# hanruihua/NeuPAN

Measured on AMD Instinct MI355X. Metric: MPC plans/sec (node), diff robot, 1k pts, T=10, K=10; ctrl L2 vs ref, higher is better.
Workload: dtype f32; 1 GPU; BASELINE.json configs[1]: batch=256 synthetic scenes/GPU, diff robot, 1000 pts, T=10, K=10 (iter_threshold=0), M=10, fp32 DUNE (MFMA) + fp64 QP; scenes_per_gpu=256, points=1000, T=10, K=10, M=10, batches_in_flight=40, chains=8, issue_threads=8

## Files before the change

### neupan_amd/csrc/create.hip

```cpp
#include "handle.h"
#include "launch.h"

#include <algorithm>
#include <cmath>
#include <cstdio>
#include <cstdlib>
#include <cstring>
#include <map>

static std::mutex g_pack_mu;
static std::map<std::string, std::weak_ptr<SharedPack>> g_packs;
static long long g_pack_calibrations = 0, g_pack_hits = 0;

struct CalibKnobDef { const char* name; void (*parse)(const char* v, CalibKnobs& k); };
static Precision parse_precision(const char* v) {
  return !strcmp(v, "bf16") ? Precision::bf16 : (!strcmp(v, "fp32") ? Precision::fp32 : Precision::invalid);
}
static const CalibKnobDef kCalibKnobs[] = {
    {"NPA_DUNE_FP32KEYS", [](const char*, CalibKnobs& k) { k.forced_mode = 0; }},
    {"NPA_KEY_TERMS", [](const char* v, CalibKnobs& k) { const int t = atoi(v); if (k.forced_mode != 0 && (t == 1 || t == 3 || t == 4)) k.forced_mode = t; }},
    {"NPA_KEY_SAFETY", [](const char* v, CalibKnobs& k) { const double s = atof(v); if (s >= 1.0 && s <= 1e3) k.key_safety = s; }},
    {"NPA_GEO_GRID", [](const char* v, CalibKnobs& k) { const int n = atoi(v); if (n >= 64 && n <= 8192) k.geo_grid = n / 8 * 8; }},
    {"NPA_GEO_NOCHECK", [](const char*, CalibKnobs& k) { k.geo_nocheck = true; }},
    {"NPA_GEO_TABLE", [](const char* v, CalibKnobs& k) { k.geo_table = atoi(v) != 0; }},
    {"NPA_KTAB_SAFETY", [](const char* v, CalibKnobs& k) { const double s = atof(v); if (s >= 1.0 && s <= 100.0) k.ktab_safety = s; }},
    {"NPA_KEYS_PRECISION", [](const char* v, CalibKnobs& k) { k.keys_precision = parse_precision(v); }},
    {"NPA_K16_SAFETY", [](const char* v, CalibKnobs& k) { const double s = atof(v); if (s >= 1.0 && s <= 100.0) k.k16_safety = s; }},
    {"NPA_ROWS_PRECISION", [](const char* v, CalibKnobs& k) { k.rows_precision = parse_precision(v); }},
};

struct Knobs {
  CalibKnobs calib;
  std::string calib_key;
  bool sel_debug = false, qp_cold = false, qp_generic = false, skip_selftest = false, pack_cache = true;
  bool qp_order = true;
  double audit_rate = 1.0 / 64.0;
  float margin_scale = 1.f;
};

static Knobs read_knobs() {
  Knobs k;
  for (const CalibKnobDef& d : kCalibKnobs) {
    const char* v = getenv(d.name);
    k.calib_key.push_back('|');
    if (v) { k.calib_key.append(v); d.parse(v, k.calib); } else k.calib_key.push_back('\x01');
  }
  k.sel_debug = getenv("NPA_SEL_DEBUG") != nullptr;
  k.qp_cold = getenv("NPA_QP_COLD") != nullptr;
  k.qp_generic = getenv("NPA_QP_GENERIC") != nullptr;
  if (const char* env = getenv("NPA_QP_ORDER")) k.qp_order = atoi(env) != 0;
  k.skip_selftest = getenv("NPA_SKIP_SELFTEST") != nullptr;
  if (const char* env = getenv("NPA_PACK_CACHE")) k.pack_cache = atoi(env) != 0;
  if (const char* env = getenv("NPA_AUDIT_RATE")) { double v = atof(env); if (v >= 0.0 && v <= 1.0) k.audit_rate = v; }
  if (const char* env = getenv("NPA_GEO_MARGIN_SCALE")) { double v = atof(env); if (v > 0.0 && v <= 100.0) k.margin_scale = (float)v; }
  return k;
}

#ifdef NPA_EXPERIMENTS
static void read_experiment_knobs(npa_handle* h) { h->select_v1 = getenv("NPA_SELECT_V1") != nullptr; }
#endif


template <class T>
struct DevScratch {
  T* p = nullptr;
  hipError_t alloc_zeroed(size_t n) {
    hipError_t e = hipMalloc(&p, n * sizeof(T));
    return e == hipSuccess ? hipMemset(p, 0, n * sizeof(T)) : e;
  }
  ~DevScratch() { if (p) (void)hipFree(p); }
};

static void set_calibrated(DevParams& P, const Calibration& c) { P.geo_rcal = c.geo_rcal; P.geo_far = c.geo_far; P.geo_tab = c.geo_tab; }

static void use_key_mode(npa_handle* h) { h->key_terms = h->cal.key_terms; h->key_err = h->cal.key_err; h->key_e0 = h->cal.key_e0; }
static void apply_calibration(npa_handle* h, const Calibration& c) {
  h->cal = c;
  set_calibrated(h->P, c);
  use_key_mode(h);
}

static constexpr int kBandsPadded = (NPA_GEO_BANDS + 3) & ~3;
static const float kCalibHalves[3] = {8.f, 32.f, 128.f};

static void band_margins(const float* raw, const bool* seen, double safety, float floor, float* margin, float* near) {
  for (int bnd = 0; bnd < NPA_GEO_BANDS; ++bnd) {
    float m = -1.f;
    for (int q = std::max(bnd - 1, 0); q <= std::min(bnd + 1, NPA_GEO_BANDS - 1); ++q)
      if (seen[q]) m = std::max(m, raw[q]);
    near[bnd] = m;
    margin[bnd] = (m < 0.f || !(m < 1e30f)) ? INFINITY : std::max((float)(safety * m), floor);
  }
}

static void residual_margins(const unsigned* bits, double safety, float floor, float (&margin)[kBandsPadded], float& worst_err,
                             float& worst_margin) {
  float raw[NPA_GEO_BANDS], near[NPA_GEO_BANDS];
  bool seen[NPA_GEO_BANDS];
  for (int bnd = 0; bnd < NPA_GEO_BANDS; ++bnd) { memcpy(&raw[bnd], &bits[bnd], 4); seen[bnd] = bits[bnd] != 0u; }
  for (int bnd = 0; bnd < kBandsPadded; ++bnd) margin[bnd] = INFINITY;
  band_margins(raw, seen, safety, floor, margin, near);
  worst_err = 0.f; worst_margin = 0.f;
  for (int bnd = 0; bnd <= npa_geo_band(8.0f) && bnd < NPA_GEO_BANDS; ++bnd)
    if (near[bnd] >= 0.f) { worst_err = std::max(worst_err, near[bnd]); worst_margin = std::max(worst_margin, margin[bnd]); }
}

static hipError_t calibrate_network_keys(const DevParams& P, const float* wpack, const CalibKnobs& k, int forced, Calibration& c) {
  const int modes[2] = {1, 3};
  const float floor_e0[2] = {1e-4f, 2e-5f}, cap_e0[2] = {5e-2f, 1e-3f};
  bool ok[2] = {false, false};
  const double sf = k.key_safety > 0 ? k.key_safety : 5.0;
  DevScratch<unsigned> dmax;
  hipError_t e = hipMalloc(&dmax.p, sizeof(unsigned));
  for (int m = 0; m < 2 && e == hipSuccess; ++m) {
    if (forced > 0 && forced != modes[m]) continue;
    unsigned bits = 0;
    e = hipMemset(dmax.p, 0, sizeof(unsigned));
    if (e == hipSuccess) e = npa_launch_key_calib(P, wpack, modes[m], 1024, 25.0f, dmax.p, nullptr);
    if (e == hipSuccess) e = hipMemcpy(&bits, dmax.p, sizeof(unsigned), hipMemcpyDeviceToHost);
    if (e != hipSuccess) break;
    float err;
    memcpy(&err, &bits, sizeof(err));
    c.err_mode[m] = err;
    c.e0_mode[m] = std::max((float)(sf * err), floor_e0[m]);
    ok[m] = c.e0_mode[m] <= cap_e0[m] || forced == modes[m];
  }
  if (e != hipSuccess) return e;
  const int pick = ok[0] ? 0 : (ok[1] ? 1 : -1);
  c.key_terms = 0; c.key_err = 0.f; c.key_e0 = 0.f;
  if (pick >= 0) { c.key_terms = modes[pick]; c.key_err = c.err_mode[pick]; c.key_e0 = c.e0_mode[pick]; }
  c.key_auto = forced < 0 && ok[0] && ok[1];
  return hipSuccess;
}
// ... 190 lines not shown
  if (cfg->receding < 1 || cfg->receding > NPA_MAX_T) return fail(NPA_E_UNSUPPORTED, "receding outside [1,NPA_MAX_T]");
  if (cfg->nrmp_max_num < 0 || cfg->nrmp_max_num > NPA_MAX_M) return fail(NPA_E_UNSUPPORTED, "nrmp_max_num outside [0,NPA_MAX_M]");
  if (cfg->edge_num < 3 || cfg->edge_num > NPA_MAX_E) return fail(NPA_E_UNSUPPORTED, "edge_num outside [3,NPA_MAX_E]");
  if (cfg->kinematics < 0 || cfg->kinematics > 2) return fail(NPA_E_ARG, "unknown kinematics");
  if (cfg->iter_num < 1) return fail(NPA_E_ARG, "iter_num < 1");
  if (npa_qp_shmem_bytes(cfg->receding, cfg->nrmp_max_num) > 160 * 1024) return fail(NPA_E_UNSUPPORTED, "T*M too large for LDS");
  need_w = cfg->nrmp_max_num > 0 && cfg->dune_max_num > 0;
  if (need_w && !w) return fail(NPA_E_ARG, "DUNE weights required unless nrmp_max_num == 0 or dune_max_num == 0");
  P.T = cfg->receding; P.M = (cfg->dune_max_num > 0) ? cfg->nrmp_max_num : 0; P.E = cfg->edge_num;
  P.kin = cfg->kinematics; P.K = cfg->iter_num; P.dune_max_num = cfg->dune_max_num;
  {
    long long n = cfg->dune_max_num > 0 ? cfg->dune_max_num : 1;
    if (n > NPA_MAX_POINTS) n = NPA_MAX_POINTS;
    P.key_stride = (int)((n + 31) / 32 * 32);
  }
  P.iter_threshold = cfg->iter_threshold;
  P.dt = cfg->step_time; P.dt32 = (float)cfg->step_time; P.L = cfg->wheelbase;
  for (int k = 0; k < 2; ++k) { P.speed_bound[k] = cfg->speed_bound[k]; P.acce_bound[k] = cfg->acce_bound[k]; }
  P.ro_obs = cfg->ro_obs; P.bk = cfg->bk;
  for (int k = 0; k < 3; ++k) P.q_s[k] = cfg->q_s[k];
  P.p_u = cfg->p_u; P.eta = cfg->eta; P.d_max = cfg->d_max; P.d_min = cfg->d_min;
  for (int e = 0; e < NPA_MAX_E; ++e) { P.G[e][0] = cfg->G[e][0]; P.G[e][1] = cfg->G[e][1]; P.h[e] = cfg->h[e]; }
  geo_valid = npa_polygon_geometry(P);
  return NPA_OK;
}

extern "C" int npa_dbg_pack_image(const npa_config* cfg, const npa_dune_weights* w, float* image, size_t image_floats, void* params,
                                  size_t params_bytes, size_t* params_size, int* geo_valid, size_t* offsets, int n_offsets) {
  if (!cfg) return fail(NPA_E_ARG, "npa_dbg_pack_image: null configuration");
  const size_t off[13] = {WP_W1, WP_WL, WP_VEC, WP_W6, WP_B6, WP_BF, WP_WLS, WP_WB16, WP_TABH, WP_W116, WP_WL16, WP_VEC16, WP_TOTAL};
  for (int i = 0; offsets && i < n_offsets && i < 13; ++i) offsets[i] = off[i];
  if (params_size) *params_size = sizeof(DevParams);
  DevParams P;
  memset(&P, 0, sizeof(P));
  bool need_w = false, valid = false;
  if (int rc = params_from_config(cfg, w, P, need_w, valid)) return rc;
  if (geo_valid) *geo_valid = valid ? 1 : 0;
  if (params) memcpy(params, &P, std::min(params_bytes, sizeof(P)));
  if (image) {
    std::vector<float> img;
    npa_build_pack_image(P, valid, need_w ? w : nullptr, img);
    memcpy(image, img.data(), std::min(image_floats, img.size()) * sizeof(float));
  }
  return NPA_OK;
}

static hipError_t audit_block_reset(npa_handle* h) {
  if (!h->audit_dev) return hipSuccess;
  unsigned blk[8] = {0, 0, 0, 0, 0, 0, 0, 0};
  void* mirror = nullptr;
  if (h->audit_host && hipHostGetDevicePointer(&mirror, h->audit_host, 0) != hipSuccess) mirror = nullptr;
  memcpy(&blk[6], &mirror, sizeof(mirror));
  if (h->audit_host) *(volatile unsigned*)h->audit_host = 0;
  return hipMemcpy(h->audit_dev, blk, sizeof(blk), hipMemcpyHostToDevice);
}

static hipError_t alloc_handle_buffers(npa_handle* h) {
  hipError_t e = hipMalloc(&h->sel_stats_dev, 4 * sizeof(unsigned));
  if (e == hipSuccess) e = hipMemset(h->sel_stats_dev, 0, 4 * sizeof(unsigned));
  if (e == hipSuccess) e = hipHostMalloc(&h->sel_stats_host, sizeof(unsigned), hipHostMallocDefault);
  if (e == hipSuccess) *h->sel_stats_host = 0;
  if (e == hipSuccess) e = hipMalloc(&h->audit_dev, 8 * sizeof(unsigned));
  if (e == hipSuccess) e = hipHostMalloc(&h->audit_host, sizeof(unsigned), hipHostMallocMapped);
  if (e == hipSuccess) e = audit_block_reset(h);
  return e;
}

static int npa_self_test(npa_handle* h);

static int create_handle(npa_handle* h, bool need_w, const npa_dune_weights* w) {
  std::vector<float> image;
  npa_build_pack_image(h->P, h->geo_valid, need_w ? w : nullptr, image);
  const Knobs knobs = read_knobs();
  h->knobs = knobs.calib;
  h->sel_debug = knobs.sel_debug; h->qp_warm = !knobs.qp_cold; h->qp_generic = knobs.qp_generic;
  h->qp_order = knobs.qp_order;
#ifdef NPA_EXPERIMENTS
  read_experiment_knobs(h);
#endif
  if (int rc = hip_status(hipGetDevice(&h->device))) return rc;
  hipDeviceProp_t prop;
  if (hipGetDeviceProperties(&prop, h->device) == hipSuccess && prop.multiProcessorCount > 0) h->n_cu = prop.multiProcessorCount;
  if (int rc = acquire_pack(h, image, need_w, knobs)) return rc;
  if (need_w) {
    if (int rc = hip_status(alloc_handle_buffers(h))) return rc;
    h->audit_thresh = knobs.audit_rate >= 1.0 ? 0xFFFFFFFFu : (unsigned)(knobs.audit_rate * 4294967296.0);
    h->margin_scale = knobs.margin_scale;
  }
  return knobs.skip_selftest ? NPA_OK : npa_self_test(h);
}

extern "C" int npa_create(const npa_config* cfg, const npa_dune_weights* w, npa_handle** out) {
  if (!cfg || !out) return fail(NPA_E_ARG, "npa_create: null argument");
  DevParams P;
  memset(&P, 0, sizeof(P));
  bool need_w = false, geo_valid = false;
  if (int rc = params_from_config(cfg, w, P, need_w, geo_valid)) return rc;
  npa_handle* h = new npa_handle();
  memcpy(&h->P, &P, sizeof(P));
  h->geo_valid = geo_valid;
  const int rc = create_handle(h, need_w, w);
  if (rc != NPA_OK) {
    const std::string msg = g_err;
    npa_destroy(h);
    return fail(rc, msg);
  }
  *out = h;
  return NPA_OK;
}

extern "C" int npa_destroy(npa_handle* h) {
  if (!h) return NPA_OK;
  {
    int cur = -1;
    if (hipGetDevice(&cur) == hipSuccess) {
      if (cur != h->device) (void)hipSetDevice(h->device);
      (void)hipDeviceSynchronize();
      if (cur != h->device) (void)hipSetDevice(cur);
    }
    (void)hipGetLastError();
  }
  for (auto& p : h->ev_dune) { hipEventDestroy(p.a); hipEventDestroy(p.b); }
  for (auto& p : h->ev_sel) { hipEventDestroy(p.a); hipEventDestroy(p.b); }
  for (auto& p : h->ev_qp) { hipEventDestroy(p.a); hipEventDestroy(p.b); }
  h->wpack = nullptr;
  {
    std::lock_guard<std::mutex> lk(g_pack_mu);
    h->pack.reset();
  }
  if (h->sel_stats_dev) hipFree(h->sel_stats_dev);
  if (h->sel_stats_host) hipHostFree(h->sel_stats_host);
  if (h->audit_dev) hipFree(h->audit_dev);
  if (h->audit_host) hipHostFree(h->audit_host);
  if (h->stage_cand) hipFree(h->stage_cand);
  delete h;
  return NPA_OK;
}

extern "C" int npa_key_mode(const npa_handle* h, int* key_terms, float* measured_error, float* margin_e0) {
  if (!h) return fail(NPA_E_ARG, "npa_key_mode: null handle");
  if (key_terms) *key_terms = h->key_terms;
  if (measured_error) *measured_error = h->key_err;
  if (margin_e0) *margin_e0 = h->key_e0;
  return NPA_OK;
}

extern "C" int npa_pack_cache_stats(int64_t* calibrations, int64_t* shared_creates, int64_t* alive) {
  std::lock_guard<std::mutex> lk(g_pack_mu);
  if (calibrations) *calibrations = g_pack_calibrations;
  if (shared_creates) *shared_creates = g_pack_hits;
  if (alive) {
    int64_t n = 0;
    for (auto& kv : g_packs) n += kv.second.expired() ? 0 : 1;
    *alive = n;
  }
  return NPA_OK;
}

extern "C" int npa_geo_report(const npa_handle* h, float* out, int n) {
  if (!h || !out || n < 1) return fail(NPA_E_ARG, "npa_geo_report: bad argument");
  const Calibration& c = h->cal;
  const float v[10] = {h->geo_valid ? 1.f : 0.f, c.geo_err, c.geo_margin, c.geo_refine, c.geo_slope, h->P.geo_far,
                       c.keys_bf16 ? c.k16_err : 0.f, c.keys_bf16 ? c.k16_margin : 0.f,
                       h->P.geo_tab ? c.ktab_err : 0.f, h->P.geo_tab ? c.ktab_margin : 0.f};
  for (int i = 0; i < n && i < 10; ++i) out[i] = v[i];
  return NPA_OK;
// ... 235 lines not shown
```

### neupan_amd/csrc/dune_device.h

```cpp
#pragma once

typedef float f32x16 __attribute__((ext_vector_type(16)));

#define DUNE_THREADS 256
#define DUNE_WAVES 4

#define WSYNC()                                              \
  do {                                                       \
    __builtin_amdgcn_fence(__ATOMIC_SEQ_CST, "wavefront");   \
    __builtin_amdgcn_wave_barrier();                         \
  } while (0)

__device__ __forceinline__ float pair_sum(float x) {
  auto r = __builtin_amdgcn_permlane32_swap(__float_as_uint(x), __float_as_uint(x), false, false);
  return __uint_as_float(r[0]) + __uint_as_float(r[1]);
}

__device__ __forceinline__ float tanh_scaled(float y) {
  float e = __builtin_amdgcn_exp2f(y);
  return fmaf(-2.0f, __builtin_amdgcn_rcpf(e + 1.0f), 1.0f);
}

__device__ __forceinline__ void load_vec16(const float* v, int hf, float out[16]) {
#pragma unroll
// ... 989 lines not shown
    for (int e = 0; e < E; ++e) {
      const float rx = x - P.pvx[e], ry = y - P.pvy[e];
      inside = inside && (fmaf(P.pdy[e], rx, -(P.pdx[e] * ry)) <= 0.f);
      float t = fmaf(rx, P.pdx[e], ry * P.pdy[e]) * P.pil[e];
      t = fminf(fmaxf(t, 0.f), 1.f);
      const float qx = fmaf(-t, P.pdx[e], rx), qy = fmaf(-t, P.pdy[e], ry);
      best = fminf(best, fmaf(qx, qx, qy * qy));
    }
    return inside ? 0.f : __builtin_amdgcn_sqrtf(best);
  }
}
template <int E, class PP>
__device__ __forceinline__ float geo_key(const PP& P, float x, float y) {
  return P.geo_rect ? geo_key_t<E, true>(P, x, y) : geo_key_t<E, false>(P, x, y);
}

__device__ __forceinline__ float geo_tab_corr(const float* __restrict__ wpack, float x, float y) {
  const float cx = wpack[WP_TABH], cy = wpack[WP_TABH + 1], h0 = wpack[WP_TABH + 2], inv0 = wpack[WP_TABH + 3];
  const float rx = x - cx, ry = y - cy;
  const float a = fmaxf(fabsf(rx), fabsf(ry));
  const int lvl = a < h0 ? 0 : (a < 4.0f * h0 ? 1 : (a < 16.0f * h0 ? 2 : 3));
  const float sc = lvl == 0 ? 1.0f : (lvl == 1 ? 4.0f : (lvl == 2 ? 16.0f : 64.0f));
  const float half = h0 * sc, inv = inv0 * (1.0f / sc);
  const float fx = fminf(fmaxf((rx + half) * inv, 0.f), (float)NPA_TAB_N - 0.001f);
  const float fy = fminf(fmaxf((ry + half) * inv, 0.f), (float)NPA_TAB_N - 0.001f);
  const int ix = (int)fx, iy = (int)fy;
  const float tx = fx - (float)ix, ty = fy - (float)iy;
  const uint2 c = reinterpret_cast<const uint2*>(wpack + WP_TAB)[((size_t)lvl * NPA_TAB_N + iy) * NPA_TAB_N + ix];
  typedef _Float16 h2_t __attribute__((ext_vector_type(2)));
  union { unsigned u; h2_t h; } lo, hi;
  lo.u = c.x; hi.u = c.y;
  const float f00 = (float)lo.h[0], f10 = (float)lo.h[1], f01 = (float)hi.h[0], f11 = (float)hi.h[1];
  const float r0 = fmaf(tx, f10 - f00, f00), r1 = fmaf(tx, f11 - f01, f01);
  return fmaf(ty, r1 - r0, r0);
}

#define SEL2_TRIP 256
template <int E, bool RECT, bool VEL, bool DEC>
__device__ __forceinline__ unsigned key_pass(const DevParams& P, const SliceFrame& F, const float* px_row, const float* py_row,
                                             const float* vx_row, const float* vy_row, unsigned* dkey, int n_raw, int n_use,
                                             int n_pad, int lane) {
  const __amdgpu_buffer_rsrc_t rx = __builtin_amdgcn_make_buffer_rsrc(const_cast<float*>(px_row), 0, n_raw * 4, 0x00020000);
  const __amdgpu_buffer_rsrc_t ry = __builtin_amdgcn_make_buffer_rsrc(const_cast<float*>(py_row), 0, n_raw * 4, 0x00020000);
  const __amdgpu_buffer_rsrc_t rvx = __builtin_amdgcn_make_buffer_rsrc(const_cast<float*>(VEL ? vx_row : px_row), 0, n_raw * 4, 0x00020000);
  const __amdgpu_buffer_rsrc_t rvy = __builtin_amdgcn_make_buffer_rsrc(const_cast<float*>(VEL ? vy_row : py_row), 0, n_raw * 4, 0x00020000);
  const float tdt = F.tstep;
  unsigned lmin = 0xFFFFFFFFu;
  for (int n0 = 0; n0 < n_pad; n0 += SEL2_TRIP) {
    float gx[4], gy[4], vx[4], vy[4];
#pragma unroll
    for (int u = 0; u < 4; ++u) {
      const int n = n0 + lane + 64 * u;
      unsigned off = (unsigned)n * 4u;
      if constexpr (DEC) off = (unsigned)src_index(n < n_use ? n : n_use - 1, n_raw, n_use) * 4u;
      gx[u] = __uint_as_float(__builtin_amdgcn_raw_buffer_load_b32(rx, off, 0, 0));
      gy[u] = __uint_as_float(__builtin_amdgcn_raw_buffer_load_b32(ry, off, 0, 0));
      if constexpr (VEL) {
        vx[u] = __uint_as_float(__builtin_amdgcn_raw_buffer_load_b32(rvx, off, 0, 0));
        vy[u] = __uint_as_float(__builtin_amdgcn_raw_buffer_load_b32(rvy, off, 0, 0));
      }
    }
#pragma unroll
    for (int u = 0; u < 4; ++u) {
      const int n = n0 + lane + 64 * u;
      float x = gx[u], y = gy[u];
      if constexpr (VEL) {
        x = __fadd_rn(x, __fmul_rn(tdt, __fmul_rn(vx[u], P.dt32)));
        y = __fadd_rn(y, __fmul_rn(tdt, __fmul_rn(vy[u], P.dt32)));
      }
      const float dx = x - F.tx, dy = y - F.ty;
      const float p0x = fmaf(F.c, dx, F.s * dy), p0y = fmaf(F.c, dy, -(F.s * dx));
      unsigned k = __float_as_uint(geo_key_t<E, RECT>(P, p0x, p0y));
      k = n < n_use ? k : 0xFFFFFFFFu;
      dkey[n] = k;
      lmin = min(lmin, k);
    }
  }
  return lmin;
}

#define SEL_OPAQUE_V(x) asm volatile("" : "+v"(x))
#define SEL_OPAQUE_S(x) do { (x) = __builtin_amdgcn_readfirstlane(x); asm volatile("" : "+s"(x)); } while (0)
#define SEL_LDS_FRAME (6 * NPA_MAX_E)
enum { ST_OVERFLOW = 1, ST_ALL = 2, ST_USE16 = 4, ST_USET = 8, ST_AUD16 = 16, ST_AUDIT_WAVE = 32, ST_HAS_AUDIT = 64, ST_DISTRUST = 128 };
#define ST_IS(f) ((st & (unsigned)(f)) != 0u)
#define ST_PUT(f, v) (st = (v) ? (st | (unsigned)(f)) : (st & ~(unsigned)(f)))
#define SEL2_TRIP 256
#ifdef NPA_SEL_PROF
#define SELP_WAVES 4096
__device__ unsigned long long npa_sel_prof[SELP_WAVES][16];
extern "C" int npa_dbg_sel_prof(unsigned long long* out16, int reset) {
  static unsigned long long host[SELP_WAVES][16];
  if (out16) {
    if (hipMemcpyFromSymbol(host, HIP_SYMBOL(npa_sel_prof), sizeof(host)) != hipSuccess) return -1;
    for (int i = 0; i < 16; ++i) { out16[i] = 0; for (int w = 0; w < SELP_WAVES; ++w) out16[i] += host[w][i]; }
  }
  if (reset) {
    memset(host, 0, sizeof(host));
    if (hipMemcpyToSymbol(HIP_SYMBOL(npa_sel_prof), host, sizeof(host)) != hipSuccess) return -1;
  }
  return 0;
}
#define SELP_DECL unsigned long long spt_ = __builtin_amdgcn_s_memtime(), sacc_[11] = {0, 0, 0, 0, 0, 0, 0, 0, 0, 0, 0}; const unsigned long long sp0_ = spt_
#define SELP(i) do { const unsigned long long n_ = __builtin_amdgcn_s_memtime(); sacc_[i] += n_ - spt_; spt_ = n_; } while (0)
#else
#define SELP_DECL
#define SELP(i)
#endif
#define NPA_KARG __attribute__((address_space(4)))
#define NPA_GLOBAL __attribute__((address_space(1)))
typedef const char NPA_KARG* karg_ptr;
struct SelGeoArgs {
  DevParams P; const float* wpack; int n_stride; const float* cur_s; const float* points; const float* vel; const int* n_points;
  const int* flags; float* mu_sorted; float* lam_sorted; float* pts_sorted; float* dist_sorted; int* count; int scene0, t0, nsl,
  nscene, debug; unsigned* stats; const float* trig; unsigned* audit; unsigned audit_thresh, audit_seed; float margin_scale;
};
struct SelGeoGroupArgs { DevParams P; SelGeoGroup G; int t0, nsl, nscene, debug; unsigned audit_thresh; float margin_scale; };
struct SelOutPtrs { float* mu; float* lam; float* pts; float* dist; int* count; };
static_assert(offsetof(SelGeoArgs, count) - offsetof(SelGeoArgs, mu_sorted) == 32 && offsetof(SelGeoCall, count) - offsetof(SelGeoCall, mu_sorted) == 32,
              "SelOutPtrs is read as one block");
static_assert(sizeof(DevParams) == 0x1a8 && offsetof(SelGeoArgs, wpack) == sizeof(DevParams) && offsetof(SelGeoGroupArgs, G) == sizeof(DevParams),
              "DevParams is the first argument of both kernels");
static_assert(sizeof(SelGeoCall) == 0x78 && sizeof(SelGeoGroupArgs) == 0x1a8 + 8 * 0x78 + 24 && offsetof(SelGeoGroupArgs, debug) == 0x1a8 + 8 * 0x78 + 12,
              "SelGeoGroupArgs mirrors select_geo_group_kernel(P, G, t0, nsl, nscene, debug, audit_thresh, margin_scale)");
static_assert(offsetof(SelGeoArgs, mu_sorted) == 0x1a8 + 0x38 && offsetof(SelGeoArgs, debug) == 0x1a8 + 0x70 && offsetof(SelGeoArgs, stats) == 0x1a8 + 0x78 &&
              offsetof(SelGeoArgs, audit) == 0x1a8 + 0x88 && sizeof(SelGeoArgs) == 0x1a8 + 0xa0,
              "SelGeoArgs mirrors the parameter list of select_geo_kernel");
__device__ __forceinline__ karg_ptr karg_fence(karg_ptr p) { asm volatile("" : "+s"(p)); return p; }
template <class T>
__device__ __forceinline__ T karg_load(karg_ptr p, size_t off) { return *reinterpret_cast<const T NPA_KARG*>(p + off); }
#define SEL_KARG(T_, member) karg_load<T_>(SEL_KARGS_LATE(), SEL_KARG_OFF(member))
template <int E>
__device__ __forceinline__ float geo_key_karg(karg_ptr kbase, float x, float y) {
  return geo_key<E>(*reinterpret_cast<const DevParams NPA_KARG*>(karg_fence(kbase)), x, y);
}

template <int E, bool BF16 = false, bool KEYS16 = false>
__global__ __attribute__((amdgpu_flat_work_group_size(64, 64), amdgpu_waves_per_eu(E <= 6 ? 4 : 3, E <= 6 ? 4 : 3))) void select_geo_kernel(
    DevParams P, const float* __restrict__ wpack, int n_stride, const float* __restrict__ cur_s,
    const float* __restrict__ points, const float* __restrict__ vel, const int* __restrict__ n_points,
    const int* __restrict__ flags, float* __restrict__ mu_sorted_, float* __restrict__ lam_sorted_,
    float* __restrict__ pts_sorted_, float* __restrict__ dist_sorted_, int* __restrict__ count_, int scene0, int t0, int nsl,
    int nscene, int debug, unsigned* __restrict__ stats_, const float* __restrict__ trig, unsigned* __restrict__ audit,
    unsigned audit_thresh, unsigned audit_seed, float margin_scale) {
#define SEL_KARG_OFF(member) offsetof(SelGeoArgs, member)
#define SEL_KBASE_OFF(member) offsetof(SelGeoArgs, member)
  const karg_ptr sel_kbase = (karg_ptr)__builtin_amdgcn_kernarg_segment_ptr();
#define SEL_KARGS_LATE() karg_fence(sel_kbase)
#define SEL_KOFF_STORE()
#define SEL_KOFF() 0
#include "select_geo_carve.inc"
  int lane = threadIdx.x;
  SELP_DECL;
  const int w = blockIdx.x, xcd = w & 7, r_ = w >> 3;
  const int bl = (r_ / nsl) * 8 + xcd;
  if (bl >= nscene) return;
  const int t = r_ % nsl + t0, b = bl + scene0;
#include "select_geo_body.inc"
#undef SEL_KARG_OFF
#undef SEL_KBASE_OFF
#undef SEL_KARGS_LATE
#undef SEL_KOFF_STORE
#undef SEL_KOFF
}

template <int E, bool BF16 = false, bool KEYS16 = false>
__global__ __attribute__((amdgpu_flat_work_group_size(64, 64), amdgpu_waves_per_eu(E <= 6 ? 4 : 3, E <= 6 ? 4 : 3))) void select_geo_group_kernel(
// ... 34 lines not shown
```

### neupan_amd/csrc/pan_common.h

```cpp
#pragma once
#include <hip/hip_runtime.h>
#include <stdint.h>
#include <atomic>

#define NPA_MAX_T 21
#define NPA_MAX_M 32
#define NPA_MAX_E 8
#define NPA_MAX_POINTS 32768

struct NpaDeviceOnce {
  std::atomic<unsigned long long> mask{0};
  bool need(int* dev_out) {
    int d = 0;
    if (hipGetDevice(&d) != hipSuccess) d = 0;
    *dev_out = d;
    return !(mask.load(std::memory_order_acquire) & (1ull << (d & 63)));
  }
  void done(int d) { mask.fetch_or(1ull << (d & 63), std::memory_order_release); }
};

struct DevParams {
  int T, M, E, kin, K, dune_max_num;
  int key_stride;
  float iter_threshold;
  float dt32;
  double dt, L;
  double speed_bound[2], acce_bound[2];
  double ro_obs, bk;
  float q_s[3], p_u, eta, d_max, d_min;
  float G[NPA_MAX_E][2];
  float h[NPA_MAX_E];
  float pvx[NPA_MAX_E], pvy[NPA_MAX_E], pdx[NPA_MAX_E], pdy[NPA_MAX_E], pil[NPA_MAX_E];
  float geo_rcal;
  float geo_far;
  int geo_rect;
  float rcx, rcy, rhx, rhy;
  int qp_aset;
  int geo_tab;
};

#define NPA_GROUP_MAX 8
struct SelGeoCall {
  const float* wpack; const float* cur_s; const float* points; const float* vel; const int* n_points; const int* flags;
  float* mu_sorted; float* lam_sorted; float* pts_sorted; float* dist_sorted; int* count; unsigned* stats; const float* trig;
  unsigned* audit; int n_stride; unsigned audit_seed;
};
struct SelGeoGroup { SelGeoCall c[NPA_GROUP_MAX]; };
struct QpSched { const int* in_cnt; const int* in_list; int* out_cnt; int* out_list; int* ticket; };
struct QpCall {
  const float* cur_s_in; const float* cur_u_in; const float* ref_s; const float* ref_us; const float* mu_sorted;
  const float* lam_sorted; const float* pts_sorted; const float* dist_sorted; const int* count; float* cur_s_out;
  float* cur_u_out; float* cur_d_out; float* out_s; float* out_u; float* out_d; float* out_min_distance; int* out_iters;
  float* out_nrmp_points; int* flags; float* state; double* qp_info; double* warm; float* trig_out;
  const float* theta;
  QpSched sched;
};
struct QpGroup { QpCall c[NPA_GROUP_MAX]; };
struct QpBackward {
  const float* grad_s;
  const float* grad_u;
  const float* grad_d;
  float* grad_theta;
  float* grad_nom_s;
  float* dbg_abc;
  float* dbg_f;
  double* dbg_x;
};
struct StageCall {
  float* cur_s; const float* nom_s; float* cur_u; const float* nom_u; int* flags; int* count; int* state; float* trig;
  int* sched_cnt;
};
struct StageGroup { StageCall c[NPA_GROUP_MAX]; };

#define NPA_GEO_BANDS 88
#define NPA_GEO_KEY_FAR 0x7F800000u
__host__ __device__ inline int npa_geo_band(float g) {
  union { float f; unsigned u; } v;
  v.f = g + 0.25f;
  if (v.u & 0x80000000u) return 0;
  const int b = (int)(v.u >> 20) - (int)(0x3E800000u >> 20);
  return b < 0 ? 0 : (b >= NPA_GEO_BANDS ? NPA_GEO_BANDS - 1 : b);
}

#define WP_W1 0
#define WP_WL (WP_W1 + 64)
#define WP_VEC (WP_WL + 4 * 16 * 64)
#define WP_W6 (WP_VEC + 11 * 32)
#define WP_B6 (WP_W6 + 8 * 32)
#define WP_BF (WP_B6 + 8)
#define WP_BF_FLOATS (4 * 2 * 2 * 64 * 4)
#define WP_KVEC (WP_BF + WP_BF_FLOATS)
#define WP_KSC (WP_KVEC + 5 * 32)
#define WP_KW1 (WP_KSC + 8)
#define WP_KEY_LDS_FLOATS (WP_BF_FLOATS + 5 * 32 + 8)
#define WP_GEO (WP_KW1 + 64)
#define WP_WLS (((WP_GEO + NPA_GEO_BANDS) + 3) & ~3)
#define WP_WB16 (WP_WLS + 4 * 64 * 16)
#define WP_WB16_FLOATS (4 * 2 * 64 * 4)
#define WP_K16 (WP_WB16 + WP_WB16_FLOATS)
#define WP_KTAB (WP_K16 + ((NPA_GEO_BANDS + 3) & ~3))
#define WP_TABH (WP_KTAB + ((NPA_GEO_BANDS + 3) & ~3))
#define WP_W116 (WP_TABH + 8)
#define WP_WL16 (WP_W116 + 2 * 64)
#define WP_VEC16 (WP_WL16 + 4 * 64 * 16)
#define WP_VEC16_FLOATS (11 * 32 + 8 * 32 + 8)
#define WP_TOTAL (WP_VEC16 + WP_VEC16_FLOATS)
#define NPA_TAB_KEY_FAR 0xFFFFFFFDu
#define NPA_TAB_N 512
#define NPA_TAB_LEVELS 4
#define NPA_TAB_HALF0 2.0f
#define WP_TAB ((WP_TOTAL + 3) & ~3)
#define WP_TAB_FLOATS (NPA_TAB_LEVELS * NPA_TAB_N * NPA_TAB_N * 2)
enum { V_B1 = 0, V_G1, V_BE1, V_B2, V_B3, V_G2, V_BE2, V_B4, V_B5, V_G3, V_BE3 };

__host__ __device__ inline int npa_feat(int r, int hf) { return (r & 3) + 8 * (r >> 2) + 4 * hf; }
__host__ __device__ inline int npa_feat16(int s, int kq) { return 8 * (s >> 1) + 2 * (s & 1) + (kq >> 1) + 4 * (kq & 1); }

__host__ __device__ inline size_t npa_state_floats(int T, int M, int E) {
  return (size_t)3 * (T + 1) + 2 * T + (size_t)(T + 1) * M * E + (size_t)(T + 1) * M * 2 + 4;
}

__device__ inline void npa_trig(float th, float& c, float& s) {
// ... 38 lines not shown
```

### neupan_amd/csrc/select_geo_body.inc

```
  const int T = P.T, M = P.M;
  constexpr bool TILE16 = !BF16 && !KEYS16;
  if (flags && flags[b * 4 + 0]) return;
  int n_raw = n_points ? n_points[b] : n_stride;
  n_raw = n_raw < 0 ? 0 : (n_raw > n_stride ? n_stride : n_raw);
  int n_use = n_raw < P.dune_max_num ? n_raw : P.dune_max_num;
  int orow_v = b;
  asm volatile("" : "+v"(orow_v));
  orow_v = orow_v * (T + 1) + t;
  int koff_v = SEL_KOFF();
  asm volatile("" : "+v"(koff_v));
  if (n_use <= 0) {
    if (lane == 0) ((int NPA_GLOBAL*)karg_load<int*>(karg_fence(sel_kbase) + __builtin_amdgcn_readfirstlane(koff_v), SEL_KARG_OFF(count)))[orow_v] = 0;
    return;
  }
  constexpr int NVEC = 11 * 32 + 8 * 32 + 8, NVT = (NVEC + 63) / 64, NGT = (NPA_GEO_BANDS + 63) / 64;
  float pre_v[NVT], pre_g[NGT];
#pragma unroll
  for (int i = 0; i < NVT; ++i) { const int k = lane + 64 * i; pre_v[i] = wpack[(TILE16 ? WP_VEC16 : WP_VEC) + (k < NVEC ? k : NVEC - 1)]; }
#pragma unroll
  for (int i = 0; i < NGT; ++i) { const int k = lane + 64 * i; pre_g[i] = wpack[WP_GEO + (k < NPA_GEO_BANDS ? k : NPA_GEO_BANDS - 1)]; }
  unsigned aud_viol = 0, aud_launches = 0;
  if (audit) {
    aud_viol = __hip_atomic_load(audit + 2, __ATOMIC_RELAXED, __HIP_MEMORY_SCOPE_AGENT);
    aud_launches = __hip_atomic_load(audit + 4, __ATOMIC_RELAXED, __HIP_MEMORY_SCOPE_AGENT);
// ... 43 lines not shown
    else {
      float mm = 0.f;
      for (int bb = npa_geo_band(g), be = npa_geo_band(g + boxS); bb <= be; ++bb) mm = max_nc(mm, etab[bb]);
      hi = g + boxS + mm;
    }
  }
  const float U = wave_max_f32(hi);
  unsigned thr = 0xFFFFFFFEu;
  if (!distrust && U < 3.0e38f) {
    float gs = 0.f;
#pragma unroll
    for (int rep = 0; rep < 2; ++rep) {
      const int bnd = lane + 64 * rep;
      if (bnd < NPA_GEO_BANDS) {
        const float lo_b = __uint_as_float((unsigned)(bnd + (0x3E800000u >> 20)) << 20) - 0.25f;
        const float hi_b = bnd == NPA_GEO_BANDS - 1 ? P.geo_far : __uint_as_float((unsigned)(bnd + 1 + (0x3E800000u >> 20)) << 20) - 0.25f;
        const float reach = U + etab[bnd];
        if (lo_b < P.geo_far && lo_b <= reach) gs = max_nc(gs, min_nc(hi_b, reach));
      }
    }
    gs = wave_max_f32(gs);
    thr = gs < 3.0e38f ? __float_as_uint(gs) : 0xFFFFFFFEu;
  }
  SELP(2);
  int ntot = 0;
  for (int n0 = 0; n0 < n_pad; n0 += SEL2_TRIP) {
    const uint4 k4 = *reinterpret_cast<const uint4*>(dkey + n0 + 4 * lane);
    const unsigned kk[4] = {k4.x, k4.y, k4.z, k4.w};
    bool hit[4];
#pragma unroll
    for (int u = 0; u < 4; ++u) hit[u] = kk[u] <= thr || (kk[u] - far_thr) < (0xFFFFFFFFu - far_thr);
#pragma unroll
    for (int u = 0; u < 4; ++u) {
      const unsigned long long bal = __ballot(hit[u]);
      const int pos = ntot + __builtin_amdgcn_mbcnt_hi((unsigned)(bal >> 32), __builtin_amdgcn_mbcnt_lo((unsigned)bal, 0));
      if (hit[u]) dkey[pos] = (unsigned)(n0 + 4 * lane + u);
      ntot += __popcll(bal);
    }
  }
  WSYNC();
  SELP(3);
  int ncand = ntot, fellback = 0;
  unsigned st = (has_audit ? (unsigned)ST_HAS_AUDIT : 0u) | (distrust ? (unsigned)ST_DISTRUST : 0u);
  int total = 0;
  if (ntot <= SEL_CAP && ntot >= msel) {
    if (lane < ntot) sel[lane] = (int)dkey[lane];
    WSYNC();
  } else if (ntot < msel) {
    ST_PUT(ST_OVERFLOW, true); fellback = 1; ST_PUT(ST_ALL, true); total = n_use;
  } else {
    ST_PUT(ST_OVERFLOW, true);
    fellback = 1;
    ST_PUT(ST_ALL, 2 * ntot > n_use);
    total = ST_IS(ST_ALL) ? n_use : ntot;
  }
  unsigned* ckey = dkey + ntot;
  auto cand_index = [&](int q) { return ST_IS(ST_ALL) ? q : (int)dkey[q]; };
  auto extract = [&]() {
    for (int m = 0; m < msel; ++m) {
      unsigned long long best = ~0ull;
      for (int n = lane; n < n_use; n += 64) best = umin64(best, ((unsigned long long)dkey[n] << 32) | (unsigned)n);
      best = wave_min_u64(best);
      const int idx = (int)(best & 0xFFFFFFFFu);
      if (lane == 0) { sel[m] = idx; skey[m] = (unsigned)(best >> 32); dkey[idx] = 0xFFFFFFFFu; }
      WSYNC();
    }
  };
  if (audit && audit_thresh) {
    audit_seed += (unsigned)__builtin_amdgcn_readfirstlane((int)aud_launches);
    if (blockIdx.x == 0 && lane == 0) atomicAdd(audit + 4, 1u);
    unsigned hsh = (audit_seed * 0x9E3779B1u) ^ ((unsigned)b * 0x85EBCA77u) ^ ((unsigned)t * 0xC2B2AE3Du);
    hsh ^= hsh >> 15; hsh *= 0x2C1B3C6Du; hsh ^= hsh >> 12; hsh *= 0x297A2D39u; hsh ^= hsh >> 15;
    ST_PUT(ST_AUDIT_WAVE, hsh < audit_thresh || audit_thresh == 0xFFFFFFFFu);
    if (lane == 0) frg[5 * NPA_MAX_E + 6] = __uint_as_float(audit_seed + (unsigned)t);
  }
  int viol = 0;
  float worst = 0.f;
  ST_PUT(ST_USE16, KEYS16 && ST_IS(ST_OVERFLOW) && !ST_IS(ST_ALL) && !ST_IS(ST_DISTRUST) && total > 128);
  constexpr bool TABF = !BF16 && !KEYS16 && (E == 4 || E == 8);
  ST_PUT(ST_USET, TABF && P.geo_tab != 0 && !ST_IS(ST_DISTRUST) && ntot >= msel && (ST_IS(ST_OVERFLOW) || ntot > 32));
  if (ST_IS(ST_USET) && !ST_IS(ST_OVERFLOW)) total = ntot;
  ST_PUT(ST_AUD16, false);
  float m16 = 0.f;
  SELP(4);
#pragma unroll 1
  for (int stage = (ST_IS(ST_OVERFLOW) || ST_IS(ST_USET)) ? 0 : 1;;) {
    SEL_OPAQUE_V(lane); SEL_OPAQUE_S(n_use); SEL_OPAQUE_S(n_raw); SEL_OPAQUE_S(msel);
    const int cnt = stage == 0 ? total : (stage == 1 ? ncand : (n_use < 32 ? n_use : 32));
    if (TABF && stage == 0 && ST_IS(ST_USET)) {
      unsigned* fk = ST_IS(ST_ALL) ? dkey : ckey;
#pragma unroll 1
      for (int q0 = 0; q0 < cnt; q0 += 64) {
        const int q = q0 + lane, qc = q < cnt ? q : cnt - 1;
        const int src = src_index(cand_index(qc), n_raw, n_use);
        SliceFrame Fl;
        Fl.c = frg[5 * NPA_MAX_E + 0]; Fl.s = frg[5 * NPA_MAX_E + 1];
        Fl.tx = frg[5 * NPA_MAX_E + 2]; Fl.ty = frg[5 * NPA_MAX_E + 3]; Fl.tstep = frg[5 * NPA_MAX_E + 4];
        float gx, gy, p0x, p0y;
        slice_point(P, Fl, px_row, vx_row, n_stride, src, gx, gy, p0x, p0y);
        const float gk = geo_key_karg<E>(sel_kbase, p0x, p0y);
        const unsigned kc = gk < P.geo_far ? ordered_key(gk + geo_tab_corr(wpack, p0x, p0y)) : NPA_TAB_KEY_FAR;
        if (q < cnt) fk[q] = kc;
      }
    } else
#pragma unroll 1
    for (int q0 = 0, tw = 32; q0 < cnt; q0 += tw) {
      const bool narrow = TILE16 && cnt - q0 <= 16;
      tw = narrow ? 16 : 32;
      const bool own = lane < tw;
      const int q = q0 + (lane & (tw - 1)), qc = q < cnt ? q : cnt - 1;
      int idx;
      if (stage == 0) idx = cand_index(qc);
      else if (stage == 1) idx = sel[qc];
      else {
        const int step = n_use >> 5;
        idx = step > 0 ? qc * step + (int)(__float_as_uint(frg[5 * NPA_MAX_E + 6]) % (unsigned)step) : qc;
      }
      float mu[E], gx, gy, lx = 0.f, ly = 0.f, dist = 0.f, p0x, p0y;
      SliceFrame Fl;
      Fl.c = frg[5 * NPA_MAX_E + 0]; Fl.s = frg[5 * NPA_MAX_E + 1];
      Fl.tx = frg[5 * NPA_MAX_E + 2]; Fl.ty = frg[5 * NPA_MAX_E + 3]; Fl.tstep = frg[5 * NPA_MAX_E + 4];
      slice_point(P, Fl, px_row, vx_row, n_stride, src_index(idx, n_raw, n_use), gx, gy, p0x, p0y);
      if constexpr (KEYS16) {
        if (stage == 0 && ST_IS(ST_USE16)) encode_tile_bf16<E>(w1, wpack + WP_WB16, vec, w6, b6, p0x, p0y, lane, mu);
        else encode_tile_stream<E, false>(w1, wls, vec, w6, b6, p0x, p0y, lane, mu);
      } else if constexpr (TILE16) {
        if (narrow) encode_tile16_stream<E>(w1a, w1b, wls16, vec, w6, b6, p0x, p0y, lane, mu);
        else encode_tile_stream<E, true>(w1, wls, vec, w6, b6, p0x, p0y, lane, mu);
      } else if constexpr (BF16) encode_tile_bf16<E>(w1, wls, vec, w6, b6, p0x, p0y, lane, mu);
      else encode_tile_stream<E, false>(w1, wls, vec, w6, b6, p0x, p0y, lane, mu);
#pragma unroll
      for (int e = 0; e < E; ++e) {
        lx = fmaf(frg[e], mu[e], lx);
        ly = fmaf(frg[NPA_MAX_E + e], mu[e], ly);
        const float tmp = __fsub_rn(fmaf(frg[2 * NPA_MAX_E + e], p0x, __fmul_rn(frg[3 * NPA_MAX_E + e], p0y)), frg[4 * NPA_MAX_E + e]);
        dist = fmaf(mu[e], tmp, dist);
      }
      if constexpr (KEYS16 || TABF) {
        if (stage == 1 && ST_IS(ST_AUD16)) {
          const unsigned k16 = s16[qc];
          const float d16 = __uint_as_float((k16 & 0x80000000u) ? (k16 & 0x7FFFFFFFu) : ~k16);
          const float ex = fabsf(dist - d16) - (TABF ? wpack_at(wpack, WP_KTAB + npa_geo_band(d16)) * margin_scale : m16);
          const bool bad = own && q < cnt && ex > 0.f;
          viol += bad ? 1 : 0;
          worst = bad ? max_nc(worst, ex) : worst;
        }
      }
      if (stage != 0 && ST_IS(ST_HAS_AUDIT)) {
        const float g = geo_key_karg<E>(sel_kbase, p0x, p0y);
        const float ex = fabsf(dist - g) - etab[npa_geo_band(g)];
        const bool bad = own && q < cnt && g < P.geo_far && ex > 0.f;
        viol += bad ? 1 : 0;
        worst = bad ? max_nc(worst, ex) : worst;
        if constexpr (TABF) {
          if (ST_IS(ST_AUDIT_WAVE) && karg_load<int>(karg_fence(sel_kbase), offsetof(DevParams, geo_tab)) != 0) {
            const float tk = g + geo_tab_corr(wpack, p0x, p0y);
            const float mt = wpack_at(wpack, WP_KTAB + npa_geo_band(tk)) * margin_scale;
            const float ext = fabsf(dist - tk) - mt;
            const bool badt = own && q < cnt && g < P.geo_far && mt < 3.0e38f && ext > 0.f;
            viol += badt ? 1 : 0;
            worst = badt ? max_nc(worst, ext) : worst;
          }
        }
      }
      if (own && q < cnt) {
        const unsigned k = ordered_key(dist);
        if (stage == 0) {
          if (ST_IS(ST_ALL)) dkey[idx] = k;
          else ckey[q] = k;
        } else if (stage == 1) {
          float* r = rows + q * ROW_W;
#pragma unroll
          for (int e = 0; e < E; ++e) r[e] = mu[e];
          r[E] = lx; r[E + 1] = ly; r[E + 2] = gx; r[E + 3] = gy; r[E + 4] = dist;
          rkey[2 * q] = (unsigned)idx; rkey[2 * q + 1] = k;
        }
      }
    }
    WSYNC();
    if (stage == 0) SELP(5); else if (stage == 1) SELP(6); else SELP(7);
    if (stage == 2) break;
    if (stage == 1) {
      const size_t orow = (size_t)__float_as_int(frg[5 * NPA_MAX_E + 5]);
      const int Me = karg_load<int>(karg_fence(sel_kbase), offsetof(DevParams, M));
      const bool mine = lane < ncand;
      const unsigned long long kx = mine ? (((unsigned long long)rkey[2 * lane + 1] << 32) | rkey[2 * lane]) : ~0ull;
      const karg_ptr ko = SEL_KARGS_LATE() + SEL_KARG_OFF(mu_sorted);
      const SelOutPtrs O = {karg_load<float*>(ko, 0), karg_load<float*>(ko, 8), karg_load<float*>(ko, 16), karg_load<float*>(ko, 24),
                            karg_load<int*>(ko, 32)};
      int rank = 0;
      for (int i = 0; i < ncand; i += 4) {
        const unsigned long long k0 = readlane_u64(kx, i), k1 = readlane_u64(kx, (i + 1) & 63), k2 = readlane_u64(kx, (i + 2) & 63),
                                 k3 = readlane_u64(kx, (i + 3) & 63);
        rank += (k0 < kx ? 1 : 0) + (k1 < kx ? 1 : 0) + (k2 < kx ? 1 : 0) + (k3 < kx ? 1 : 0);
      }
      if (mine && rank < msel) {
        const float* r = rows + lane * ROW_W;
        float NPA_GLOBAL* mu_sorted = (float NPA_GLOBAL*)O.mu; float NPA_GLOBAL* lam_sorted = (float NPA_GLOBAL*)O.lam;
        float NPA_GLOBAL* pts_sorted = (float NPA_GLOBAL*)O.pts; float NPA_GLOBAL* dist_sorted = (float NPA_GLOBAL*)O.dist;
        auto put = [&](int q) {
          const size_t o = orow * Me + q;
#pragma unroll
          for (int e = 0; e < E; ++e) mu_sorted[o * E + e] = r[e];
          lam_sorted[o * 2 + 0] = r[E]; lam_sorted[o * 2 + 1] = r[E + 1];
          pts_sorted[o * 2 + 0] = r[E + 2]; pts_sorted[o * 2 + 1] = r[E + 3];
          dist_sorted[o] = r[E + 4];
        };
        put(rank);
        if (rank == 0)
#pragma unroll 1
          for (int q = msel; q < Me; ++q) put(q);
      }
      if (lane == 0) {
        int word = msel;
        if (karg_load<int>(karg_fence(sel_kbase), SEL_KBASE_OFF(debug))) {
          int nt = ntot;
          asm volatile("" : "+s"(nt));
          word |= ((nt < 255 ? nt : 255) << 8) | (fellback << 16);
        }
        ((int NPA_GLOBAL*)O.count)[orow] = word;
      }
      SELP(8);
      if (!ST_IS(ST_AUDIT_WAVE)) break;
      stage = 2;
      continue;
    }
    SEL_OPAQUE_S(st);
    const bool filt = (KEYS16 && ST_IS(ST_USE16)) || (TABF && ST_IS(ST_USET));
    if (lane == 0 && !(TABF && ST_IS(ST_USET))) {
      unsigned* stats = SEL_KARG(unsigned*, stats);
      if (stats) atomicAdd(stats, (unsigned)((total + 31) / 32));
    }
    if (ST_IS(ST_ALL) && !filt) {
      extract();
    } else if (filt) {
      const unsigned* fk = ST_IS(ST_ALL) ? dkey : ckey;
      auto key_float = [](unsigned k) { return __uint_as_float((k & 0x80000000u) ? (k & 0x7FFFFFFFu) : ~k); };
      float kt0 = 0.f, kt1 = 0.f, Ub = -3.0e38f;
      if constexpr (TABF) {
        kt0 = wpack_at(wpack, WP_KTAB + lane) * margin_scale;
        kt1 = wpack_at(wpack, WP_KTAB + 64 + (lane < NPA_GEO_BANDS - 64 ? lane : NPA_GEO_BANDS - 65)) * margin_scale;
      }
      unsigned long long prev = 0ull;
      for (int m2 = 0; m2 < msel; ++m2) {
        unsigned long long best = ~0ull;
        for (int q = lane; q < total; q += 64) {
          const unsigned long long v = ((unsigned long long)fk[q] << 32) | (unsigned)cand_index(q);
          if (v < best && (m2 == 0 || v > prev)) best = v;
        }
        prev = wave_min_u64(best);
        if constexpr (TABF) {
          const float km = key_float((unsigned)(prev >> 32));
          const int bm = __builtin_amdgcn_readfirstlane(npa_geo_band(km));
          const float mb = __uint_as_float(bm < 64 ? __builtin_amdgcn_readlane(__float_as_uint(kt0), bm & 63)
                                                   : __builtin_amdgcn_readlane(__float_as_uint(kt1), bm & 63));
          Ub = max_nc(Ub, km + mb);
          if (!(km == km)) Ub = __builtin_inff();
        }
      }
      const unsigned kth = (unsigned)(prev >> 32);
      const float dk = key_float(kth);
      bool bound_ok;
      unsigned thr16, thr_hi = NPA_TAB_KEY_FAR;
      if constexpr (TABF) {
        float gs = -3.0e38f;
// ... 127 lines not shown
```

Before: 893,700 plans/s.

## Add first-tile selection path: encode 16 best table candidates, prune rest by bound

When the geo table is enabled and the candidate count is between 17 and 32 with msel <= 16, candidates are ranked by table key and only the top 16 are run through the full DUNE encode in stage 1. The remaining candidates are kept only if their lower bound (table key minus a per-band margin) does not exceed the msel-th exact distance. The survivors are then encoded in a second pass that starts at offset 16. This cuts the network evaluations per wave in the common case, at the cost of extra LDS ranking, wave syncs and a possible second pass, and selection correctness now depends on the margin bounds.

```diff
diff --git a/neupan_amd/csrc/create.hip b/neupan_amd/csrc/create.hip
--- a/neupan_amd/csrc/create.hip
+++ b/neupan_amd/csrc/create.hip
@@ -34,6 +34,7 @@
   std::string calib_key;
   bool sel_debug = false, qp_cold = false, qp_generic = false, skip_selftest = false, pack_cache = true;
   bool qp_order = true;
+  bool sel_first_tile = true;
   double audit_rate = 1.0 / 64.0;
   float margin_scale = 1.f;
 };
@@ -49,6 +50,7 @@
   k.qp_cold = getenv("NPA_QP_COLD") != nullptr;
   k.qp_generic = getenv("NPA_QP_GENERIC") != nullptr;
   if (const char* env = getenv("NPA_QP_ORDER")) k.qp_order = atoi(env) != 0;
+  if (const char* env = getenv("NPA_SEL_FIRST_TILE")) k.sel_first_tile = atoi(env) != 0;
   k.skip_selftest = getenv("NPA_SKIP_SELFTEST") != nullptr;
   if (const char* env = getenv("NPA_PACK_CACHE")) k.pack_cache = atoi(env) != 0;
   if (const char* env = getenv("NPA_AUDIT_RATE")) { double v = atof(env); if (v >= 0.0 && v <= 1.0) k.audit_rate = v; }
@@ -405,6 +407,7 @@
   hipDeviceProp_t prop;
   if (hipGetDeviceProperties(&prop, h->device) == hipSuccess && prop.multiProcessorCount > 0) h->n_cu = prop.multiProcessorCount;
   if (int rc = acquire_pack(h, image, need_w, knobs)) return rc;
+  if (h->P.geo_tab && knobs.sel_first_tile) h->P.geo_tab |= NPA_GEO_TAB_FIRST_TILE;
   if (need_w) {
     if (int rc = hip_status(alloc_handle_buffers(h))) return rc;
     h->audit_thresh = knobs.audit_rate >= 1.0 ? 0xFFFFFFFFu : (unsigned)(knobs.audit_rate * 4294967296.0);
diff --git a/neupan_amd/csrc/dune_device.h b/neupan_amd/csrc/dune_device.h
--- a/neupan_amd/csrc/dune_device.h
+++ b/neupan_amd/csrc/dune_device.h
@@ -1095,7 +1095,8 @@
 #define SEL_OPAQUE_V(x) asm volatile("" : "+v"(x))
 #define SEL_OPAQUE_S(x) do { (x) = __builtin_amdgcn_readfirstlane(x); asm volatile("" : "+s"(x)); } while (0)
 #define SEL_LDS_FRAME (6 * NPA_MAX_E)
-enum { ST_OVERFLOW = 1, ST_ALL = 2, ST_USE16 = 4, ST_USET = 8, ST_AUD16 = 16, ST_AUDIT_WAVE = 32, ST_HAS_AUDIT = 64, ST_DISTRUST = 128 };
+enum { ST_OVERFLOW = 1, ST_ALL = 2, ST_USE16 = 4, ST_USET = 8, ST_AUD16 = 16, ST_AUDIT_WAVE = 32, ST_HAS_AUDIT = 64, ST_DISTRUST = 128,
+       ST_FIRST = 256, ST_SECOND = 512 };
 #define ST_IS(f) ((st & (unsigned)(f)) != 0u)
 #define ST_PUT(f, v) (st = (v) ? (st | (unsigned)(f)) : (st & ~(unsigned)(f)))
 #define SEL2_TRIP 256
diff --git a/neupan_amd/csrc/pan_common.h b/neupan_amd/csrc/pan_common.h
--- a/neupan_amd/csrc/pan_common.h
+++ b/neupan_amd/csrc/pan_common.h
@@ -38,6 +38,7 @@
   int qp_aset;
   int geo_tab;
 };
+#define NPA_GEO_TAB_FIRST_TILE 2
 
 #define NPA_GROUP_MAX 8
 struct SelGeoCall {
diff --git a/neupan_amd/csrc/select_geo_body.inc b/neupan_amd/csrc/select_geo_body.inc
--- a/neupan_amd/csrc/select_geo_body.inc
+++ b/neupan_amd/csrc/select_geo_body.inc
@@ -149,29 +149,64 @@
   if (ST_IS(ST_USET) && !ST_IS(ST_OVERFLOW)) total = ntot;
   ST_PUT(ST_AUD16, false);
   float m16 = 0.f;
+  static_assert(SEL_CAP >= 32 && NPA_MAX_M >= 32, "the first-tile path ranks up to 32 candidates into sel[], s16[] and skey[]");
+  if constexpr (TABF) {
+    if ((P.geo_tab & NPA_GEO_TAB_FIRST_TILE) != 0 && !ST_IS(ST_DISTRUST) && !ST_IS(ST_AUDIT_WAVE) && msel <= 16 && ntot > 16 && ntot <= 32) {
+      ST_PUT(ST_FIRST, true);
+      total = ntot;
+    }
+  }
   SELP(4);
 #pragma unroll 1
-  for (int stage = (ST_IS(ST_OVERFLOW) || ST_IS(ST_USET)) ? 0 : 1;;) {
+  for (int stage = (ST_IS(ST_OVERFLOW) || ST_IS(ST_USET) || ST_IS(ST_FIRST)) ? 0 : 1;;) {
     SEL_OPAQUE_V(lane); SEL_OPAQUE_S(n_use); SEL_OPAQUE_S(n_raw); SEL_OPAQUE_S(msel);
     const int cnt = stage == 0 ? total : (stage == 1 ? ncand : (n_use < 32 ? n_use : 32));
-    if (TABF && stage == 0 && ST_IS(ST_USET)) {
+    if (TABF && stage == 0 && (ST_IS(ST_USET) || ST_IS(ST_FIRST))) {
       unsigned* fk = ST_IS(ST_ALL) ? dkey : ckey;
+      const bool first = (__builtin_amdgcn_readfirstlane((int)st) & ST_FIRST) != 0;
 #pragma unroll 1
       for (int q0 = 0; q0 < cnt; q0 += 64) {
         const int q = q0 + lane, qc = q < cnt ? q : cnt - 1;
-        const int src = src_index(cand_index(qc), n_raw, n_use);
+        const int iq = cand_index(qc);
+        const int src = src_index(iq, n_raw, n_use);
         SliceFrame Fl;
         Fl.c = frg[5 * NPA_MAX_E + 0]; Fl.s = frg[5 * NPA_MAX_E + 1];
         Fl.tx = frg[5 * NPA_MAX_E + 2]; Fl.ty = frg[5 * NPA_MAX_E + 3]; Fl.tstep = frg[5 * NPA_MAX_E + 4];
         float gx, gy, p0x, p0y;
         slice_point(P, Fl, px_row, vx_row, n_stride, src, gx, gy, p0x, p0y);
         const float gk = geo_key_karg<E>(sel_kbase, p0x, p0y);
-        const unsigned kc = gk < P.geo_far ? ordered_key(gk + geo_tab_corr(wpack, p0x, p0y)) : NPA_TAB_KEY_FAR;
+        const float tk = gk + geo_tab_corr(wpack, p0x, p0y);
+        int tsg = __float_as_int(tk) >> 31;
+        asm("" : "+v"(tsg));
+        const unsigned tko = tk != tk ? 0xFFFFFFFEu : ~(__float_as_uint(tk) ^ (~(unsigned)tsg >> 1));
+        const unsigned kc = gk < P.geo_far ? tko : NPA_TAB_KEY_FAR;
         if (q < cnt) fk[q] = kc;
+        if (first) {
+          const int tb = max(__float_as_int(tk + 0.25f), 0x3E800000) >> 20;
+          unsigned ti = (unsigned)min(tb + (WP_KTAB - (int)(0x3E800000u >> 20)), WP_KTAB + NPA_GEO_BANDS - 1);
+          asm("" : "+v"(ti));
+          const float mt = wpack[ti] * margin_scale;
+          const float lb = gk < P.geo_far ? tk - mt : -3.0e38f;
+          const unsigned kb = (__float_as_uint(gk) & 0x7FFFFFE0u) | (unsigned)lane | ((unsigned)((cnt - 1 - q) >> 31) >> 1);
+          if (lane < 32) s16[32 + lane] = kb;
+          WSYNC();
+          int rk = 0;
+#pragma unroll
+          for (int j = 0; j < 32; ++j) rk -= (int)(s16[32 + j] - kb) >> 31;
+          WSYNC();
+          if (q < cnt) { sel[rk] = iq; s16[rk] = kc; skey[rk] = __float_as_uint(lb); }
+        }
+      }
+      if (first) {
+        WSYNC();
+        ncand = 16;
+        stage = 1;
+        SELP(4);
+        continue;
       }
     } else
 #pragma unroll 1
-    for (int q0 = 0, tw = 32; q0 < cnt; q0 += tw) {
+    for (int q0 = TABF ? (__builtin_amdgcn_readfirstlane((int)st) & ST_SECOND) >> 5 : 0, tw = 32; q0 < cnt; q0 += tw) {
       const bool narrow = TILE16 && cnt - q0 <= 16;
       tw = narrow ? 16 : 32;
       const bool own = lane < tw;
@@ -248,6 +283,48 @@
     if (stage == 0) SELP(5); else if (stage == 1) SELP(6); else SELP(7);
     if (stage == 2) break;
     if (stage == 1) {
+      if constexpr (TABF) {
+        if ((__builtin_amdgcn_readfirstlane((int)st) & ST_FIRST) != 0) {
+          ST_PUT(ST_FIRST, false);
+          unsigned myk = rkey[2 * (lane & 15) + 1] >> 1;
+          asm volatile("" : "+v"(myk));
+          int below = 0, above = 0, j0 = 0;
+          asm volatile("" : "+v"(j0));
+#pragma unroll
+          for (int j = 0; j < 16; ++j) {
+            const unsigned kj = rkey[2 * (j0 + j) + 1] >> 1;
+            below -= (int)(kj - myk) >> 31;
+            above -= (int)(myk - kj) >> 31;
+          }
+          if (below < msel && msel <= 16 - above) skey[0] = (myk << 1) | 1u;
+          WSYNC();
+          const unsigned kM = skey[0];
+          int msg = (int)kM >> 31;
+          asm("" : "+v"(msg));
+          const float dM = __uint_as_float(~(kM ^ ((unsigned)msg >> 1)));
+          int nrest = total;
+          SEL_OPAQUE_S(nrest);
+          nrest -= 16;
+          const int j = 16 + min(lane, nrest - 1);
+          const int ij = sel[j];
+          const unsigned kj = s16[j];
+          const bool hit = lane < nrest && !(__uint_as_float(skey[j]) > dM);
+          const unsigned long long bal = __ballot(hit);
+          const int pos = 16 + __builtin_amdgcn_mbcnt_hi((unsigned)(bal >> 32), __builtin_amdgcn_mbcnt_lo((unsigned)bal, 0));
+          WSYNC();
+          if (hit) { sel[pos] = ij; s16[pos] = kj; }
+          WSYNC();
+          SELP(8);
+          fellback = 4;
+          if (bal != 0ull) {
+            fellback = 5;
+            ncand = 16 + __popcll(bal);
+            ST_PUT(ST_SECOND, true);
+            ST_PUT(ST_AUD16, true);
+            continue;
+          }
+        }
+      }
       const size_t orow = (size_t)__float_as_int(frg[5 * NPA_MAX_E + 5]);
       const int Me = karg_load<int>(karg_fence(sel_kbase), offsetof(DevParams, M));
       const bool mine = lane < ncand;
```

Measured after the change: 927,300 plans/s, median of 6. 3.8% higher.
